# AI-Application-and-Integration-Lab/RDPN6D

Measured on AMD Instinct MI355X. Metric: RGB-D crops/sec (fwd+PnP) at 256x256, higher is better.
Workload: dtype f32

## Files before the change

include/rdpn6d.h:

```cpp
#ifndef RDPN6D_H
#define RDPN6D_H

#ifdef __cplusplus
extern "C" {
#endif

#define RDPN6D_OK 0
#define RDPN6D_EINVAL -1
#define RDPN6D_EHIP -2
#define RDPN6D_ENOMEM -3

const char* rdpn6d_last_error(void);
int rdpn6d_version(void);
int rdpn6d_device_count(void);

void farthest_point_sampling(float* pts, int* idxs, int pn, int sn);
void farthest_point_sampling_init_center(float* pts, int* idxs, int pn, int sn);
int rdpn6d_fps_host(const float* pts, int* idxs, int pn, int sn, int start);
int rdpn6d_fps_device(const float* d_pts, const int* d_offsets, int nobj, int max_pn, int sn, int start,
                      int* d_idxs, float* d_mindist, void* stream);
long long rdpn6d_fps_workspace_bytes(int nobj);
int rdpn6d_fps_device_ws(const float* d_pts, const int* d_offsets, int nobj, int max_pn, int sn, int start, int* d_idxs,
                         float* d_mindist, void* workspace, long long workspace_bytes, void* stream);

// ... 28 lines not shown

int rdpn6d_conv2d_bf16(const rdpn6d_conv_desc* d, int out_f32, void* stream);
int rdpn6d_conv2d_splitk_bf16(const rdpn6d_conv_desc* d, int out_f32, int ksplit, float* workspace, void* stream);
int rdpn6d_conv2d_bf16_bnstats(const rdpn6d_conv_desc* d, double* stats, int stats_row0, int* stats_rows, void* stream);
int rdpn6d_conv2d_bf16_bnbwd(const rdpn6d_conv_desc* d, const void* bn_x, int bn_cs, int bn_co, const float* mean, const float* invstd,
                             const float* gamma, const float* beta, double* partial, int* rows, void* stream);
int rdpn6d_bn_relu_backward_apply_bf16(const void* x, int xcs, int xco, const void* dy, int dcs, int dco, const float* mean,
                                       const float* invstd, const float* gamma, const float* beta, float* dgamma, float* dbeta, void* dx,
                                       int xgcs, int xgco, long long M, int C, const double* partial, int S, void* stream);
int rdpn6d_conv2d_bf16_bnbwd_y(const rdpn6d_conv_desc* d, const void* bn_x, int bn_cs, int bn_co, const void* bn_y, int y_cs, int y_co,
                               const float* mean, const float* invstd, double* partial, int* rows, void* stream);
int rdpn6d_bn_backward_apply_bf16(const void* x, int xcs, int xco, const void* dy, int dcs, int dco, const void* y, int ycs, int yco,
                                  const float* mean, const float* invstd, const float* gamma, float* dgamma, float* dbeta, void* dx,
                                  int xgcs, int xgco, void* dres, int rcs, int rco, long long M, int C, const double* partial, int S,
                                  void* stream);
void rdpn6d_conv_bf16_force_tile(int bm, int bn);
void rdpn6d_conv_bf16_force_stages(int nst);
int rdpn6d_conv_bf16_tile_for(const rdpn6d_conv_desc* d, int* bm, int* bn);
int rdpn6d_conv_bf16_uses_pingpong(const rdpn6d_conv_desc* d, int out_f32);
int rdpn6d_split_bf16x3(const float* x, long long n, void* planes, long long plane_elems, void* stream);
int rdpn6d_conv_bf16x3_eligible(const rdpn6d_conv_desc* d);
int rdpn6d_conv_bf16x3_kernel_for(const rdpn6d_conv_desc* d);
int rdpn6d_conv2d_bf16x3(const rdpn6d_conv_desc* d, long long x_plane_elems, long long w_plane_elems, void* y_planes,
                         long long y_plane_elems, void* stream);
int rdpn6d_conv2d_bf16x3_ex(const rdpn6d_conv_desc* d, long long x_plane_elems, long long w_plane_elems, void* y_planes,
                            long long y_plane_elems, const void* res_planes, long long res_plane_elems, void* stream);
int rdpn6d_split_h2(const float* x, int src_cs, int src_co, int C, void* dst, long long npix, int* overflow_flag, void* stream);
int rdpn6d_conv_h2_kernel_for(const rdpn6d_conv_desc* d);
int rdpn6d_conv2d_h2(const rdpn6d_conv_desc* d, void* y_h2, const void* res_h2, int* overflow_flag, void* stream);
int rdpn6d_conv2d_h2_cb(const rdpn6d_conv_desc* d, void* y_h2, const void* res_h2, int* overflow_flag, const float* crop_bias,
                        void* stream);
long long rdpn6d_conv_h2_workspace_bytes(const rdpn6d_conv_desc* d);
void rdpn6d_conv_h2_set_clock_probe(unsigned long long* buf);
void rdpn6d_conv_h2_set_wfrag(int mode);
int rdpn6d_conv_h2_colmax_ok(const rdpn6d_conv_desc* d, int rows_per_group);
int rdpn6d_conv2d_h2_colmax(const rdpn6d_conv_desc* d, unsigned long long* keys, int rows_per_group, int* overflow_flag, void* stream);
int rdpn6d_h2_colmax_decode(unsigned long long* keys, int groups, int N, int Npad, void* out_h2, void* stream);
int rdpn6d_conv_h2_wfrag_wanted(const rdpn6d_conv_desc* d);
int rdpn6d_h2_weight_frag(const void* w_h2, int Npad, int ntaps, int cchunks, void* w_frag, void* stream);
int rdpn6d_conv2d_h2_wf(const rdpn6d_conv_desc* d, void* y_h2, const void* res_h2, int* overflow_flag, const void* w_frag, void* stream);
int rdpn6d_conv2d_h2_ws(const rdpn6d_conv_desc* d, void* y_h2, const void* res_h2, int* overflow_flag, const float* crop_bias,
                        void* workspace, long long workspace_bytes, void* stream);
int rdpn6d_conv_h2_fuse1x1_ok(const rdpn6d_conv_desc* d);
int rdpn6d_conv2d_h2_fuse1x1(const rdpn6d_conv_desc* d, const void* res_h2, int* overflow_flag, const float* crop_bias,
                             const void* w1_h2, const float* scale1, const float* bias1, float* out, int out_cs, int n_out,
                             void* stream);
int rdpn6d_upsample_bilinear_h2(const void* x, int B, int H, int W, int C, int factor, void* y, int* overflow_flag, void* stream);
int rdpn6d_upsample_bilinear_h2_ex(const void* x, int B, int H, int W, int C, int factor, void* y, int out_cs, int out_co, int relu,
                                   int* overflow_flag, void* stream);
int rdpn6d_xyz_subsample_h2(const float* x, int B, int xc, int R, int step, void* y, int out_cs, int out_co, int* overflow_flag,
                            void* stream);
int rdpn6d_global_max_concat_h2(void* buf, int B, int HW, int C, int cs, void* stream);
int rdpn6d_global_max_h2(const void* x_h2, int B, int HW, int C, int cs, void* gmax_h2, void* stream);
int rdpn6d_convt3x3s2_const_bias_f32(const float* V, const float* scale, int B, int F, float* out , void* stream);
int rdpn6d_stem_pool_h2(const float* x, int B, int xc, int R, const void* w_h2, const float* scale, const float* shift, void* y,
                        int* overflow_flag, void* stream);
int rdpn6d_stem_pool_h2_ex(const float* x, int B, int xc, int R, const void* w_h2, const float* scale, const float* shift, void* y,
                           int out_fmt, int* overflow_flag, void* stream);
int rdpn6d_stem_pack_h2(const float* w_oihw, void* w_h2, float* inv_scale, void* stream);
void rdpn6d_conv_bf16_force_chunk(int row_bytes);
int rdpn6d_stem_conv7x7_bf16(const float* x, int B, int xc, int R, const float* w, const float* scale,
                             const float* shift, void* y, void* stream);
int rdpn6d_maxpool3x3s2_bf16(const void* x, int B, int H, int W, int C, void* y, void* stream);
int rdpn6d_upsample_bilinear_bf16(const void* x, int B, int H, int W, int C, int factor, void* y, void* stream);
int rdpn6d_xyz_subsample_bf16(const float* x, int B, int xc, int R, int step, void* y, int out_cs, int out_co,
                              void* stream);
// ... 281 lines not shown
```

rdpn6d_amd/_lib.py:

```python
import ctypes
import os

HERE = os.path.dirname(os.path.abspath(__file__))
LIB_PATH = os.environ.get("RDPN6D_LIB") or os.path.join(HERE, "librdpn6d_hip.so")

_ll = ctypes.c_longlong
c_float_p = ctypes.c_void_p
c_int_p = ctypes.c_void_p
_vp, _i, _f, _u = ctypes.c_void_p, ctypes.c_int, ctypes.c_float, ctypes.c_uint


class ConvDesc(ctypes.Structure):

    _fields_ = [
        ("x", _vp), ("w", _vp), ("scale", _vp), ("shift", _vp), ("res", _vp), ("y", _vp),
        ("B", _i), ("H", _i), ("W", _i), ("Cin", _i), ("in_cs", _i), ("in_co", _i), ("Ho", _i), ("Wo", _i),
        ("stride", _i), ("ntaps", _i), ("dy", _i * 9), ("dx", _i * 9), ("N", _i), ("Npad", _i), ("OH", _i), ("OW", _i),
        ("osy", _i), ("osx", _i), ("ooy", _i), ("oox", _i), ("out_cs", _i), ("out_co", _i), ("res_cs", _i),
        ("res_co", _i), ("act", _i), ("slope", _f),
    ]


SIGNATURES = {
    "rdpn6d_last_error": (ctypes.c_char_p, []),
# ... 103 lines not shown
    "rdpn6d_bn_train_stats_bf16": (_i, [_vp, _ll, _i, _i, _i, _f, _f, _vp, _vp, _vp, _vp, _vp, _vp]),
    "rdpn6d_bn_apply_bf16": (_i, [_vp, _i, _i, _vp, _vp, _vp, _vp, _vp, _i, _i, _vp, _i, _i, _ll, _i, _i, _vp]),
    "rdpn6d_bn_backward_bf16": (_i, [_vp, _i, _i, _vp, _i, _i, _vp, _i, _i, _vp, _vp, _vp, _vp, _vp, _vp, _i, _i, _vp, _i, _i,
                                     _ll, _i, _i, _vp, _vp]),
    "rdpn6d_bn_relu_backward_bf16": (_i, [_vp, _i, _i, _vp, _i, _i, _vp, _vp, _vp, _vp, _vp, _vp, _vp, _i, _i, _ll, _i, _vp, _vp]),
    "rdpn6d_channel_sum_bf16": (_i, [_vp, _ll, _i, _i, _i, _vp, _i, _vp, _vp]),
    "rdpn6d_maxpool3x3s2_backward_bf16": (_i, [_vp, _vp, _i, _i, _i, _i, _vp, _vp]),
    "rdpn6d_upsample_bilinear_backward_bf16": (_i, [_vp, _i, _i, _i, _i, _i, _vp, _vp]),
    "rdpn6d_global_max_concat_backward_bf16": (_i, [_vp, _vp, _i, _i, _i, _i, _vp, _vp]),
    "rdpn6d_stem_im2col_bf16": (_i, [_vp, _i, _i, _i, _vp, _vp]),
    "rdpn6d_stem_rowpatch_bf16": (_i, [_vp, _i, _i, _i, _vp, _vp]),
    "rdpn6d_repack_f32": (_i, [_vp, _vp, _vp, _i, _vp]),
    "rdpn6d_split_h2": (_i, [_vp, _i, _i, _i, _vp, _ll, _vp, _vp]),
    "rdpn6d_conv_h2_kernel_for": (_i, [_vp]),
    "rdpn6d_conv2d_h2": (_i, [_vp, _vp, _vp, _vp, _vp]),
    "rdpn6d_upsample_bilinear_h2": (_i, [_vp, _i, _i, _i, _i, _i, _vp, _vp, _vp]),
    "rdpn6d_xyz_subsample_h2": (_i, [_vp, _i, _i, _i, _i, _vp, _i, _i, _vp, _vp]),
    "rdpn6d_stem_pool_h2": (_i, [_vp, _i, _i, _i, _vp, _vp, _vp, _vp, _vp, _vp]),
    "rdpn6d_stem_pool_h2_ex": (_i, [_vp, _i, _i, _i, _vp, _vp, _vp, _vp, _i, _vp, _vp]),
    "rdpn6d_stem_pack_h2": (_i, [_vp, _vp, _vp, _vp]),
    "rdpn6d_global_max_concat_h2": (_i, [_vp, _i, _i, _i, _i, _vp]),
    "rdpn6d_upsample_bilinear_h2_ex": (_i, [_vp, _i, _i, _i, _i, _i, _vp, _i, _i, _i, _vp, _vp]),
    "rdpn6d_global_max_h2": (_i, [_vp, _i, _i, _i, _i, _vp, _vp]),
    "rdpn6d_convt3x3s2_const_bias_f32": (_i, [_vp, _vp, _i, _i, _vp, _vp]),
    "rdpn6d_conv2d_h2_cb": (_i, [_vp, _vp, _vp, _vp, _vp, _vp]),
    "rdpn6d_conv2d_h2_ws": (_i, [_vp, _vp, _vp, _vp, _vp, _vp, ctypes.c_longlong, _vp]),
    "rdpn6d_conv_h2_fuse1x1_ok": (_i, [ctypes.POINTER(ConvDesc)]),
    "rdpn6d_conv2d_h2_fuse1x1": (_i, [ctypes.POINTER(ConvDesc), _vp, _vp, _vp, _vp, _vp, _vp, _vp, _i, _i, _vp]),
    "rdpn6d_conv_h2_workspace_bytes": (ctypes.c_longlong, [_vp]),
    "rdpn6d_conv_h2_colmax_ok": (_i, [ctypes.POINTER(ConvDesc), _i]),
    "rdpn6d_conv2d_h2_colmax": (_i, [ctypes.POINTER(ConvDesc), _vp, _i, _vp, _vp]),
    "rdpn6d_h2_colmax_decode": (_i, [_vp, _i, _i, _i, _vp, _vp]),
    "rdpn6d_conv_h2_set_wfrag": (None, [_i]),
    "rdpn6d_conv_h2_set_clock_probe": (None, [_vp]),
    "rdpn6d_conv_h2_wfrag_wanted": (_i, [ctypes.POINTER(ConvDesc)]),
    "rdpn6d_h2_weight_frag": (_i, [_vp, _i, _i, _i, _vp, _vp]),
    "rdpn6d_conv2d_h2_wf": (_i, [ctypes.POINTER(ConvDesc), _vp, _vp, _vp, _vp, _vp]),
    "rdpn6d_ransac_pnp_f32": (_i, [_vp, _vp, _vp, _vp, _vp, _i, _i, _f, _i, _f, ctypes.c_uint, _i, _f, _vp, _vp, _vp, _vp, _vp]),
    "rdpn6d_ransac_pnp_ex": (_i, [_vp, _vp, _vp, _vp, _vp, _i, _i, _f, _i, _f, ctypes.c_uint, _i, _f, _i, _vp, _vp, _vp, _vp, _vp]),
    "rdpn6d_ransac_pnp_workspace_bytes": (_ll, [_i]),
    "rdpn6d_ransac_pnp_ws": (_i, [_vp, _vp, _vp, _vp, _vp, _i, _i, _f, _i, _f, ctypes.c_uint, _i, _f, _i, _vp, _vp, _vp, _vp, _vp, _ll, _vp]),
    "rdpn6d_select_correspondences_f32": (_i, [_vp, _i, _vp, _i, _i, _i, _vp, _vp, _i, _i, _i, _i, _f, _vp, _vp, _vp, _vp, _vp, _vp]),
    "rdpn6d_select_correspondences_mt_f32": (_i, [_vp, _i, _vp, _i, _i, _i, _vp, _vp, _i, _i, _i, _i, _f, _i, _vp, _vp, _vp, _vp, _vp, _vp]),
}

for _k in [k for k in list(SIGNATURES) if "_bf16" in k and "bf16x3" not in k]:
    SIGNATURES[_k.replace("_bf16", "_fp16")] = SIGNATURES[_k]
SIGNATURES["rdpn6d_repack_fp16"] = SIGNATURES["rdpn6d_repack_f32"]

_lib = None


def load():
    global _lib
    if _lib is None:
        if not os.path.exists(LIB_PATH):
            raise RuntimeError(
                f"{LIB_PATH} is missing: build the HIP extension first (python -m rdpn6d_amd.build). "
                "rdpn6d_amd has no CPU fallback."
            )
        import torch

        if torch.cuda.device_count() > 0:
            torch.cuda.init()
        lib = ctypes.CDLL(LIB_PATH)
        for name, (res, args) in SIGNATURES.items():
# ... 12 lines not shown
```

rdpn6d_amd/csrc/conv_igemm_h2.hip:

```cpp
#include "conv_h2_common.h"

#include <cstdio>
#include <cstdlib>

#ifdef RDPN6D_PROBE
__device__ unsigned long long* g_h2_probe = nullptr;
extern "C" int rdpn6d_debug_h2_probe(void* buf)
{
    RD_CHECK_HIP(hipMemcpyToSymbol(HIP_SYMBOL(g_h2_probe), &buf, sizeof(buf)));
    return RDPN6D_OK;
}
#endif

namespace {

constexpr int HT_BYTES = 16384;
constexpr int LDS_8PH = 2 * 4 * HT_BYTES;
constexpr int LDS_8PH_FUSED = 8 * (32 * 72 * 4 + 32 * 272);
static_assert(LDS_8PH_FUSED >= LDS_8PH && LDS_8PH_FUSED <= 160 * 1024, "LDS");

template <bool FUSE, bool CMAX>
__device__ __forceinline__ void conv_h2_8ph_body(const ConvH2Args& ax)
{
    extern __shared__ __attribute__((aligned(1024))) unsigned char smem[];
// ... 412 lines not shown
        const unsigned long long t_issued = __builtin_readcyclecounter();
        asm volatile("s_waitcnt vmcnt(0)" ::: "memory");
        const unsigned long long t_done = __builtin_readcyclecounter();
        if (g_h2_probe && lane == 0) {
            unsigned long long* o = g_h2_probe + ((size_t)blockIdx.x * 8 + wave) * 8;
            o[0] = pq_loop0 - pq_start;
            o[1] = pq_loop1 - pq_loop0;
            o[2] = t_issued - pq_loop1;
            o[3] = t_done - t_issued;
            o[4] = pq_rt0;
            o[5] = __builtin_amdgcn_s_memrealtime();
            o[6] = (unsigned long long)nk;
        }
    }
#endif
}

template <bool FUSE>
__global__ __launch_bounds__(512) void conv_h2_8ph_kernel_t(const ConvH2Args ax)
{
    const bool probe = ax.clk_probe != nullptr && blockIdx.x == 0 && blockIdx.y == 0;
    unsigned long long t0 = 0, r0 = 0;
    if (probe) { t0 = __builtin_readcyclecounter(); r0 = __builtin_amdgcn_s_memrealtime(); }
    conv_h2_8ph_body<FUSE, false>(ax);
    if (probe && threadIdx.x == 0) {
        ax.clk_probe[0] = t0; ax.clk_probe[1] = r0;
        ax.clk_probe[2] = __builtin_readcyclecounter(); ax.clk_probe[3] = __builtin_amdgcn_s_memrealtime();
    }
}
__global__ __launch_bounds__(512) void conv_h2_8ph_colmax_kernel(const ConvH2Args ax) { conv_h2_8ph_body<false, true>(ax); }

constexpr auto conv_h2_8ph_kernel = conv_h2_8ph_kernel_t<false>;

template <int BM, int BN, int NST, int SCHED = 0>
__global__ __launch_bounds__(256, 2) void conv_h2_tile_kernel(const ConvH2Args ax)
{
    constexpr int NW = 4, RB = 128;
    constexpr int RPP = 1024 / RB;
    constexpr int WGN = 2, WTM = BM / 2, WTN = BN / 2;
    constexpr int TM = WTM / 32, TN = WTN / 32;
    constexpr int AG = BM / RPP / NW, BG = BN / RPP / NW;
    constexpr int NDMA = AG + BG;
    static_assert(TM >= 1 && TN >= 1 && AG >= 1 && BG >= 1, "tile / wave layout");
    extern __shared__ __attribute__((aligned(1024))) unsigned char smem[];
    unsigned char* As = smem;
    unsigned char* Bs = smem + NST * BM * RB;

    const ConvBArgs& a = ax.b;
    const rdpn6d_conv_desc& d = a.d;
    const int nblk = a.mtiles * a.ntiles;
    const int bid = blockIdx.x;
    const int q8 = nblk >> 3, r8 = nblk & 7, xcd = bid & 7, kk = bid >> 3;
    const int logical = (xcd < r8 ? xcd * (q8 + 1) : r8 * (q8 + 1) + (xcd - r8) * q8) + kk;
    const int nt = logical % a.ntiles;
    const int mt = logical / a.ntiles;
    const long long m0 = (long long)mt * BM;
    const int n0 = nt * BN;

    const int tid = threadIdx.x;
    const int lane = tid & 63;
    const int wave = __builtin_amdgcn_readfirstlane(tid >> 6);

    const int prow = lane >> 3, pslot = lane & 7;
    const unsigned px_bytes = (unsigned)d.in_cs * 4u;
    unsigned a_base[AG], a_mask[AG];
#pragma unroll
    for (int i = 0; i < AG; ++i) {
        const int row = (wave + NW * i) * RPP + prow;
        const long long m = m0 + row;
        const bool ok = m < a.M;
        const int mm = ok ? (int)m : 0;
        const int b = mm / a.HoWo;
        const int rem = mm - b * a.HoWo;
        const int oy = rem / d.Wo;
        const int ox = rem - oy * d.Wo;
        const int iy = oy * d.stride, ix = ox * d.stride;
        const int lslot = pslot ^ ((row >> 1) & 7);
        a_base[i] = (unsigned)((b * d.H + iy) * d.W + ix) * px_bytes + (unsigned)d.in_co * 4u + (unsigned)lslot * 16u;
        unsigned mask = 0;
        for (int t = 0; t < d.ntaps; ++t) {
            const int dy = (int)((a.dy_pack >> (4 * t)) & 15ull) - 8, dx = (int)((a.dx_pack >> (4 * t)) & 15ull) - 8;
            mask |= (ok && (unsigned)(iy + dy) < (unsigned)d.H && (unsigned)(ix + dx) < (unsigned)d.W) ? (1u << t) : 0u;
        }
        a_mask[i] = mask;
    }
    unsigned w_off[BG];
#pragma unroll
    for (int i = 0; i < BG; ++i) {
        const int row = (wave + NW * i) * RPP + prow;
        const int lslot = pslot ^ ((row >> 1) & 7);
        w_off[i] = (unsigned)(n0 + row) * (unsigned)a.Ktot * 4u + (unsigned)lslot * 16u;
    }
    const __amdgpu_buffer_rsrc_t xsrc = __builtin_amdgcn_make_buffer_rsrc(const_cast<float*>(d.x), 0, a.x_bytes, 0x00020000);
    const __amdgpu_buffer_rsrc_t wsrc = __builtin_amdgcn_make_buffer_rsrc(const_cast<float*>(d.w), 0, a.w_bytes, 0x00020000);

    auto stage_chunk = [&](const int tap, const int cc, const int st) {
        const int dy = (int)((a.dy_pack >> (4 * tap)) & 15ull) - 8, dx = (int)((a.dx_pack >> (4 * tap)) & 15ull) - 8;
        const unsigned toff = (unsigned)((dy * d.W + dx) * (int)px_bytes + cc * RB);
#pragma unroll
        for (int i = 0; i < AG; ++i) {
// ... 66 lines not shown
                rl[i][rr] = f16x8{};
            }
        }
    float scj[TN], shj[TN];
#pragma unroll
    for (int j = 0; j < TN; ++j) {
        const int n = nb + j * 32 + frow;
        scj[j] = (d.scale && !ax.partial) ? d.scale[n] : 1.f;
        shj[j] = (d.shift && !ax.partial) ? d.shift[n] : 0.f;
    }

    f32x16 acc[TM][TN];
#pragma unroll
    for (int i = 0; i < TM; ++i)
#pragma unroll
        for (int j = 0; j < TN; ++j)
#pragma unroll
            for (int e = 0; e < 16; ++e) acc[i][j][e] = 0.f;

    auto mma = [&](const u32x4 (&fa)[TM][4], const u32x4 (&fb)[TN][4]) {
        H2_PAIRS;
#pragma unroll
        for (int pr = 0; pr < 6; ++pr)
#pragma unroll
            for (int i = 0; i < TM; ++i)
#pragma unroll
                for (int jn = 0; jn < TN; ++jn) acc[i][jn] = h2_mfma(fa[i][H2_PA[pr]], fb[jn][H2_PB[pr]], acc[i][jn]);
    };

    u32x4 fa0[TM][4], fb0[TN][4], fa1[TM][4], fb1[TN][4];
    [[maybe_unused]] unsigned long long pr_sum[5] = {0, 0, 0, 0, 0};
    [[maybe_unused]] const unsigned long long pr_start = SCHED == 9 ? __builtin_readcyclecounter() : 0ull;
    [[maybe_unused]] const unsigned long long pr_rt0 = SCHED == 9 ? (__builtin_amdgcn_s_memrealtime() & 0xffffffffull) : 0ull;
    if constexpr (NST == 2) {
        stage_chunk(ld_tap, ld_cc, 0);
        next_chunk(ld_tap, ld_cc, ld_left, d.ntaps);
        stage_chunk(ld_tap, ld_cc, 1);
        next_chunk(ld_tap, ld_cc, ld_left, d.ntaps);
        __syncthreads();
        read_frags(0, fa0, fb0);
        __syncthreads();
        const int npairs = nk >> 1;
        for (int pr = 0; pr < npairs; ++pr) {
            stage_chunk(ld_tap, ld_cc, 0);
            next_chunk(ld_tap, ld_cc, ld_left, d.ntaps);
            read_frags(1, fa1, fb1);
            mma(fa0, fb0);
            __syncthreads();

            stage_chunk(ld_tap, ld_cc, 1);
            next_chunk(ld_tap, ld_cc, ld_left, d.ntaps);
            read_frags(0, fa0, fb0);
            mma(fa1, fb1);
            __syncthreads();
        }
        if (nk & 1) mma(fa0, fb0);
    } else {
        auto publish = [&]() {
            asm volatile("s_waitcnt vmcnt(%0) lgkmcnt(0)" ::"n"(NDMA) : "memory");
            __builtin_amdgcn_s_barrier();
            asm volatile("" ::: "memory");
        };
        stage_chunk(ld_tap, ld_cc, 0);
        next_chunk(ld_tap, ld_cc, ld_left, d.ntaps);
        stage_chunk(ld_tap, ld_cc, 1);
        next_chunk(ld_tap, ld_cc, ld_left, d.ntaps);
        stage_chunk(ld_tap, ld_cc, 2);
// ... 62 lines not shown
        const int hi = lane >> 5;
        asm volatile("s_waitcnt vmcnt(0) lgkmcnt(0)" ::: "memory");
        __builtin_amdgcn_s_barrier();
        asm volatile("" ::: "memory");
        float* cst = reinterpret_cast<float*>(smem) + wave * (32 * CS);
        if (ax.partial) {
            float* part = ax.partial + ((size_t)blockIdx.y * ax.mpad + (size_t)m0 + wm * WTM) * d.Npad + nb + c8;
#pragma unroll
            for (int i = 0; i < TM; ++i) {
#pragma unroll
                for (int j = 0; j < TN; ++j)
#pragma unroll
                    for (int e = 0; e < 16; ++e) cst[((e & 3) + 8 * (e >> 2) + 4 * hi) * CS + j * 32 + frow] = acc[i][j][e];
#pragma unroll
                for (int rr = 0; rr < 32 / RPI; ++rr) {
                    const int row = rr * RPI + rrow;
                    float* pp = part + (size_t)(i * 32 + row) * d.Npad;
                    *reinterpret_cast<f32x4*>(pp) = *reinterpret_cast<const f32x4*>(cst + row * CS + c8);
                    *reinterpret_cast<f32x4*>(pp + 4) = *reinterpret_cast<const f32x4*>(cst + row * CS + c8 + 4);
                }
            }
            return;
        }
#pragma unroll
        for (int i = 0; i < TM; ++i) {
#pragma unroll
            for (int j = 0; j < TN; ++j)
#pragma unroll
                for (int e = 0; e < 16; ++e)
                    cst[((e & 3) + 8 * (e >> 2) + 4 * hi) * CS + j * 32 + frow] = acc[i][j][e] * scj[j] + shj[j];
#pragma unroll
            for (int rr = 0; rr < NRR; ++rr) {
                const int row = rr * RPI + rrow;
                if (pixs[i][rr] >= 0) {
                    const f32x4 lo = *reinterpret_cast<const f32x4*>(cst + row * CS + c8);
                    const f32x4 hi4 = *reinterpret_cast<const f32x4*>(cst + row * CS + c8 + 4);
                    float v[8] = {lo[0], lo[1], lo[2], lo[3], hi4[0], hi4[1], hi4[2], hi4[3]};
                    if (res_pre) h2_finish_row8_t<true>(ax, v, pixs[i][rr], nb + c8, rh[i][rr], rl[i][rr]);
                    else h2_finish_row8_t<false>(ax, v, pixs[i][rr], nb + c8, rh[i][rr], rl[i][rr]);
                }
            }
        }
    }
#ifdef RDPN6D_PROBE
    if constexpr (SCHED == 9) {
        if (g_h2_probe && lane == 0) {
            const unsigned long long t_end = __builtin_readcyclecounter();
            unsigned long long* o = g_h2_probe + ((size_t)blockIdx.x * 4 + wave) * 8;
            for (int i = 0; i < 5; ++i) o[i] = pr_sum[i];
            o[5] = pr_loop_end - pr_start;
            o[6] = t_end - pr_loop_end;
            o[7] = pr_rt0 | (__builtin_amdgcn_s_memrealtime() << 32);
        }
    }
#endif
}

__global__ __launch_bounds__(256) void h2_splitk_reduce_kernel(const ConvH2Args ax)
{
    const ConvBArgs& a = ax.b;
    const rdpn6d_conv_desc& d = a.d;
    const int n8 = d.Npad >> 3;
    const long long total = a.M * n8;
    const size_t sstride = (size_t)ax.mpad * d.Npad;
    for (long long i = (long long)blockIdx.x * 256 + threadIdx.x; i < total; i += (long long)gridDim.x * 256) {
        const long long m = i / n8;
        const int ch = (int)(i - m * n8) * 8;
        if (ch >= d.N) continue;
        const float* pp = ax.partial + (size_t)m * d.Npad + ch;
        f32x4 s0 = *reinterpret_cast<const f32x4*>(pp), s1 = *reinterpret_cast<const f32x4*>(pp + 4);
        int sl = 1;
        for (; sl + 3 <= ax.nsplit; sl += 3) {
// ... 15 lines not shown
            v[q] = s0[q] * (d.scale ? d.scale[ch + q] : 1.f) + (d.shift ? d.shift[ch + q] : 0.f);
            v[4 + q] = s1[q] * (d.scale ? d.scale[ch + 4 + q] : 1.f) + (d.shift ? d.shift[ch + 4 + q] : 0.f);
        }
        h2_finish_row8(ax, v, h2_pixel_of(a, m), ch);
    }
}

template <int BM, int BN, int NST, int SCHED = 0>
int launch_h2_tile_s(const ConvH2Args& ax, hipStream_t s);
template <int BM, int BN, int NST>
int launch_h2_tile(const ConvH2Args& ax, hipStream_t s)
{
#ifdef RDPN6D_PROBE
    static const int sched = getenv("RDPN6D_H2_SCHED") ? atoi(getenv("RDPN6D_H2_SCHED")) : 0;
    if (sched == 9) return launch_h2_tile_s<BM, BN, NST, 9>(ax, s);
#endif
    return launch_h2_tile_s<BM, BN, NST, 0>(ax, s);
}
template <int BM, int BN, int NST, int SCHED>
int launch_h2_tile_s(const ConvH2Args& ax, hipStream_t s)
{
    constexpr int lds_stage = NST * (BM + BN) * 128;
    constexpr int lds_epi = 4 * 32 * (BN / 2 + 8) * 4;
    constexpr int lds = lds_stage > lds_epi ? lds_stage : lds_epi;
    static_assert(lds <= 80 * 1024 || (BM == 128 && BN == 128 && NST == 3), "two workgroups per CU (128x128 with three stages: one)");
    auto kern = conv_h2_tile_kernel<BM, BN, NST, SCHED>;
    if (lds > 64 * 1024) {
        RD_LDS_OPT_IN(kern, lds);
    }
    hipLaunchKernelGGL(kern, dim3((unsigned)(ax.b.mtiles * ax.b.ntiles), (unsigned)ax.nsplit), dim3(256), lds, s, ax);
    return RDPN6D_OK;
}

__global__ void split_h2_kernel(const float* __restrict__ x, int src_cs, int src_co, int C, _Float16* __restrict__ dst, long long npix,
                                int* __restrict__ overflow_flag)
{
    const int c8n = C >> 3;
    const long long total = npix * c8n;
    bool over = false;
    for (long long i = (long long)blockIdx.x * blockDim.x + threadIdx.x; i < total; i += (long long)gridDim.x * blockDim.x) {
        const long long p = i / c8n;
        const int c = (int)(i - p * c8n) * 8;
        const float* sp = x + p * src_cs + src_co + c;
        const f32x4 v0 = *reinterpret_cast<const f32x4*>(sp), v1 = *reinterpret_cast<const f32x4*>(sp + 4);
        const float v[8] = {v0[0], v0[1], v0[2], v0[3], v1[0], v1[1], v1[2], v1[3]};
        f16x8 hi, lo;
        float sv[8];
#pragma unroll
        for (int q = 0; q < 8; ++q) sv[q] = v[q] * H2_SCALE;
        over |= h2_split8(sv, hi, lo);
        _Float16* pp = dst + p * (2 * (long long)C) + (c >> 5) * 64 + (c & 31);
        *reinterpret_cast<f16x8*>(pp) = hi;
        *reinterpret_cast<f16x8*>(pp + 32) = lo;
    }
    if (over && overflow_flag) *overflow_flag = 1;
}

bool h2_common_ok(const rdpn6d_conv_desc* d)
{
    return d->Cin % 32 == 0 && d->in_cs % 32 == 0 && d->in_co % 32 == 0 && d->out_cs % 8 == 0 && d->out_co % 8 == 0 && d->N % 8 == 0 &&
           d->Npad % 64 == 0 && (!d->res || (d->res_cs % 4 == 0 && d->res_co % 4 == 0));
}
bool h2_big_ok(const rdpn6d_conv_desc* d)
{
    const int nk = d->ntaps * (d->Cin / 32);
    return h2_common_ok(d) && d->Npad % 256 == 0 && d->N == d->Npad && nk >= 2 && (nk & 1) == 0;
// ... 37 lines not shown

static int h2_pp_plan(const rdpn6d_conv_desc* d, long long M, int* pbm, int* pbn)
{
    static const int on = getenv("RDPN6D_H2_PP") ? atoi(getenv("RDPN6D_H2_PP")) : 1;
    static const int force = getenv("RDPN6D_H2_PP_SHAPE") ? atoi(getenv("RDPN6D_H2_PP_SHAPE")) : -1;
    if (!on || d->Npad % 128 != 0 || d->ntaps * (d->Cin / 32) < 8) return -1;
    int shape = 0;
    if ((long long)rd_cdiv(M, 256) * (d->Npad / 128) >= 224 && (long long)rd_cdiv(M, 128) * (d->Npad / 128) > 288) shape = 2;
    if (force == 0 || force == 2) shape = force;
    const int bm = shape == 0 ? 128 : 256;
    if ((long long)rd_cdiv(M, bm) * (d->Npad / 128) < 224) return -1;
    *pbm = bm;
    *pbn = 128;
    return shape;
}

static int h2_tile_ksplit(const rdpn6d_conv_desc* d, long long M, int bm, int bn)
{
    static const int off = getenv("RDPN6D_H2_NO_SPLITK") ? 1 : 0;
    const long long tiles = (long long)rd_cdiv(M, bm) * (d->Npad / bn);
    static const int tmax = getenv("RDPN6D_H2_SPLIT_TILES") ? atoi(getenv("RDPN6D_H2_SPLIT_TILES")) : 128;
    if (off || tiles >= tmax) return 0;
    const int nk = d->ntaps * (d->Cin / 32);
    int best = 0;
    for (int sl = 2; sl <= 32; sl *= 2)
        if (tiles * sl <= 512 && nk % sl == 0 && nk / sl >= 4) best = sl;
    return best;
}

static int g_h2_wfrag_mode = getenv("RDPN6D_H2_BFG") ? atoi(getenv("RDPN6D_H2_BFG")) : 0;
extern "C" void rdpn6d_conv_h2_set_wfrag(int mode) { g_h2_wfrag_mode = mode; }
static unsigned long long* g_h2_clk_probe = nullptr;
extern "C" void rdpn6d_conv_h2_set_clock_probe(unsigned long long* buf) { g_h2_clk_probe = buf; }
static bool h2_wfrag_shape_ok(int shape)
{
    const int mode = g_h2_wfrag_mode;
    return mode >= 1 && (shape == 0 || (mode >= 2 && shape == 2));
}

extern "C" int rdpn6d_conv_h2_kernel_for(const rdpn6d_conv_desc* d)
{
    if (!d || !h2_common_ok(d)) return 0;
    const long long M = (long long)d->B * d->Ho * d->Wo;
    return (h2_big_ok(d) && h2_big_pays(d, M)) ? 2 : 1;
}

extern "C" int rdpn6d_conv2d_h2_cb(const rdpn6d_conv_desc* d, void* y_h2, const void* res_h2, int* overflow_flag, const float* crop_bias,
                                   void* stream);
extern "C" int rdpn6d_conv2d_h2(const rdpn6d_conv_desc* d, void* y_h2, const void* res_h2, int* overflow_flag, void* stream)
{
    return rdpn6d_conv2d_h2_cb(d, y_h2, res_h2, overflow_flag, nullptr, stream);
}

extern "C" long long rdpn6d_conv_h2_workspace_bytes(const rdpn6d_conv_desc* d)
{
    if (!d || rdpn6d_conv_h2_kernel_for(d) != 1) return 0;
    const long long M = (long long)d->B * d->Ho * d->Wo;
    int bm, bn;
    if (h2_pp_plan(d, M, &bm, &bn) >= 0) return 0;
    h2_pick_tile(d, M, &bm, &bn);
    return (long long)h2_tile_ksplit(d, M, bm, bn) * rd_cdiv(M, bm) * bm * d->Npad * 4;
}

extern "C" int rdpn6d_conv2d_h2_ws(const rdpn6d_conv_desc* d, void* y_h2, const void* res_h2, int* overflow_flag, const float* crop_bias,
                                   void* workspace, long long workspace_bytes, void* stream);
extern "C" int rdpn6d_conv2d_h2_cb(const rdpn6d_conv_desc* d, void* y_h2, const void* res_h2, int* overflow_flag, const float* crop_bias,
                                   void* stream)
{
    return rdpn6d_conv2d_h2_ws(d, y_h2, res_h2, overflow_flag, crop_bias, nullptr, 0, stream);
}

struct H2Fuse {
    const void* w;
    const float *scale, *bias;
    float* out;
    int cs, n;
};
// ... 146 lines not shown
    for (int t = 0; t < d->ntaps; ++t) {
        RD_REQUIRE(d->dy[t] >= -8 && d->dy[t] <= 7 && d->dx[t] >= -8 && d->dx[t] <= 7, "tap offsets must be in -8..7");
        a.dy_pack |= (unsigned long long)(d->dy[t] + 8) << (4 * t);
        a.dx_pack |= (unsigned long long)(d->dx[t] + 8) << (4 * t);
    }
    a.kper = a.nk;
    a.partial = nullptr;
    hipStream_t s = (hipStream_t)stream;
    if (which == 1) {
        int bm, bn;
        const int shape = h2_pp_plan(d, a.M, &bm, &bn);
        if (shape >= 0) {
            a.mtiles = rd_cdiv(a.M, bm);
            a.ntiles = d->Npad / bn;
            ax.w_frag = h2_wfrag_shape_ok(shape) ? w_frag : nullptr;
            const int rc = conv_h2_launch_pp(ax, shape, s);
            if (rc != RDPN6D_OK) return rc;
            RD_LAUNCH_CHECK();
            return RDPN6D_OK;
        }
        h2_pick_tile(d, a.M, &bm, &bn);
        a.mtiles = rd_cdiv(a.M, bm);
        a.ntiles = d->Npad / bn;
        const int ks = h2_tile_ksplit(d, a.M, bm, bn);
        if (ks && workspace && workspace_bytes >= (long long)ks * a.mtiles * bm * d->Npad * 4) {
            ax.nsplit = ks;
            ax.mpad = a.mtiles * bm;
            ax.partial = reinterpret_cast<float*>(workspace);
            a.kper = a.nk / ks;
        }
        int rc;
        static const int nst_env = getenv("RDPN6D_H2_NST") ? atoi(getenv("RDPN6D_H2_NST")) : 0;
        const bool three = nst_env ? nst_env == 3 : a.kper >= 32;
        if (bm == 128 && bn == 128) rc = (nst_env == 3) ? launch_h2_tile<128, 128, 3>(ax, s) : launch_h2_tile<128, 128, 2>(ax, s);
        else if (bm == 128) rc = three ? launch_h2_tile<128, 64, 3>(ax, s) : launch_h2_tile<128, 64, 2>(ax, s);
        else if (bn == 128) rc = three ? launch_h2_tile<64, 128, 3>(ax, s) : launch_h2_tile<64, 128, 2>(ax, s);
        else rc = three ? launch_h2_tile<64, 64, 3>(ax, s) : launch_h2_tile<64, 64, 2>(ax, s);
        if (rc != RDPN6D_OK) return rc;
        RD_LAUNCH_CHECK();
        if (ax.partial) {
            const long long items = a.M * (d->Npad / 8);
            hipLaunchKernelGGL(h2_splitk_reduce_kernel, dim3((unsigned)((items + 255) / 256 < 4096 ? (items + 255) / 256 : 4096)), dim3(256), 0, s, ax);
            RD_LAUNCH_CHECK();
        }
        return RDPN6D_OK;
    }
    a.mtiles = rd_cdiv(a.M, 256);
    a.ntiles = d->Npad / 256;
    if (fuse && !fuse->w) {
        RD_LDS_OPT_IN(conv_h2_8ph_colmax_kernel, LDS_8PH);
        hipLaunchKernelGGL(conv_h2_8ph_colmax_kernel, dim3((unsigned)(a.mtiles * a.ntiles)), dim3(512), LDS_8PH, s, ax);
        RD_LAUNCH_CHECK();
        return RDPN6D_OK;
    }
    if (fuse) {
        RD_LDS_OPT_IN(conv_h2_8ph_kernel_t<true>, LDS_8PH_FUSED);
        hipLaunchKernelGGL(conv_h2_8ph_kernel_t<true>, dim3((unsigned)(a.mtiles * a.ntiles)), dim3(512), LDS_8PH_FUSED, s, ax);
        RD_LAUNCH_CHECK();
        return RDPN6D_OK;
    }
    RD_LDS_OPT_IN(conv_h2_8ph_kernel, LDS_8PH);
#ifdef RDPN6D_PROBE
    if (const char* e = getenv("RDPN6D_H2_ABL_A")) ax.nsplit = 100 + atoi(e);
#endif
    hipLaunchKernelGGL(conv_h2_8ph_kernel, dim3((unsigned)(a.mtiles * a.ntiles)), dim3(512), LDS_8PH, s, ax);
    RD_LAUNCH_CHECK();
// ... 3 lines not shown
```

Baseline: 9186.

## Add halo-patch staging path for 3x3 stride-1 fp16 conv tiles

Adds a patch-based variant of the tiled implicit-GEMM conv kernel for 3x3 stride-1 convs on narrow feature maps (W of 8 or 16, 64x64 tiles). For each channel chunk it loads one halo patch of input rows into double-buffered LDS, and all nine taps read shifted fragments from it, with x-boundary masking applied in registers. This replaces re-staging the A operand once per tap, cutting global loads. The cost is a more complex pipeline, per-tap masking work, and recomputing pixel indices in the epilogue.

```diff
diff --git a/include/rdpn6d.h b/include/rdpn6d.h
--- a/include/rdpn6d.h
+++ b/include/rdpn6d.h
@@ -84,6 +84,8 @@
                         void* stream);
 long long rdpn6d_conv_h2_workspace_bytes(const rdpn6d_conv_desc* d);
 void rdpn6d_conv_h2_set_clock_probe(unsigned long long* buf);
+void rdpn6d_conv_h2_set_patch(int on);
+int rdpn6d_conv_h2_patch_for(const rdpn6d_conv_desc* d);
 void rdpn6d_conv_h2_set_wfrag(int mode);
 int rdpn6d_conv_h2_colmax_ok(const rdpn6d_conv_desc* d, int rows_per_group);
 int rdpn6d_conv2d_h2_colmax(const rdpn6d_conv_desc* d, unsigned long long* keys, int rows_per_group, int* overflow_flag, void* stream);
diff --git a/rdpn6d_amd/_lib.py b/rdpn6d_amd/_lib.py
--- a/rdpn6d_amd/_lib.py
+++ b/rdpn6d_amd/_lib.py
@@ -159,6 +159,8 @@
     "rdpn6d_conv2d_h2_colmax": (_i, [ctypes.POINTER(ConvDesc), _vp, _i, _vp, _vp]),
     "rdpn6d_h2_colmax_decode": (_i, [_vp, _i, _i, _i, _vp, _vp]),
     "rdpn6d_conv_h2_set_wfrag": (None, [_i]),
+    "rdpn6d_conv_h2_set_patch": (None, [_i]),
+    "rdpn6d_conv_h2_patch_for": (_i, [ctypes.POINTER(ConvDesc)]),
     "rdpn6d_conv_h2_set_clock_probe": (None, [_vp]),
     "rdpn6d_conv_h2_wfrag_wanted": (_i, [ctypes.POINTER(ConvDesc)]),
     "rdpn6d_h2_weight_frag": (_i, [_vp, _i, _i, _i, _vp, _vp]),
diff --git a/rdpn6d_amd/csrc/conv_igemm_h2.hip b/rdpn6d_amd/csrc/conv_igemm_h2.hip
--- a/rdpn6d_amd/csrc/conv_igemm_h2.hip
+++ b/rdpn6d_amd/csrc/conv_igemm_h2.hip
@@ -468,7 +468,7 @@
 
 constexpr auto conv_h2_8ph_kernel = conv_h2_8ph_kernel_t<false>;
 
-template <int BM, int BN, int NST, int SCHED = 0>
+template <int BM, int BN, int NST, int SCHED = 0, int PW = 0>
 __global__ __launch_bounds__(256, 2) void conv_h2_tile_kernel(const ConvH2Args ax)
 {
     constexpr int NW = 4, RB = 128;
@@ -479,8 +479,9 @@
     constexpr int NDMA = AG + BG;
     static_assert(TM >= 1 && TN >= 1 && AG >= 1 && BG >= 1, "tile / wave layout");
     extern __shared__ __attribute__((aligned(1024))) unsigned char smem[];
+    constexpr int PB = PW * NW * 1024;
     unsigned char* As = smem;
-    unsigned char* Bs = smem + NST * BM * RB;
+    unsigned char* Bs = smem + (PW > 0 ? 2 * PB : NST * BM * RB);
 
     const ConvBArgs& a = ax.b;
     const rdpn6d_conv_desc& d = a.d;
@@ -499,9 +500,9 @@
 
     const int prow = lane >> 3, pslot = lane & 7;
     const unsigned px_bytes = (unsigned)d.in_cs * 4u;
-    unsigned a_base[AG], a_mask[AG];
-#pragma unroll
-    for (int i = 0; i < AG; ++i) {
+    unsigned a_base[AG] = {}, a_mask[AG] = {};
+#pragma unroll
+    for (int i = 0; i < (PW > 0 ? 0 : AG); ++i) {
         const int row = (wave + NW * i) * RPP + prow;
         const long long m = m0 + row;
         const bool ok = m < a.M;
@@ -634,7 +635,153 @@
     [[maybe_unused]] unsigned long long pr_sum[5] = {0, 0, 0, 0, 0};
     [[maybe_unused]] const unsigned long long pr_start = SCHED == 9 ? __builtin_readcyclecounter() : 0ull;
     [[maybe_unused]] const unsigned long long pr_rt0 = SCHED == 9 ? (__builtin_amdgcn_s_memrealtime() & 0xffffffffull) : 0ull;
-    if constexpr (NST == 2) {
+    if constexpr (PW > 0) {
+        constexpr int PN = PW > 0 ? PW : 1;
+        const int W = d.W;
+        const int y0 = (int)(m0 % a.HoWo) / W;
+        const bool top = y0 > 0, bot = y0 + BM / W < d.H;
+        unsigned p_off[PN];
+#pragma unroll
+        for (int i = 0; i < PN; ++i) {
+            const int p = (wave + NW * i) * RPP + prow;
+            const bool ok = p < BM + 2 * W && (p >= W || top) && (p < BM + W || bot);
+            const int lslot = pslot ^ ((p >> 1) & 7);
+            p_off[i] = ok ? (unsigned)(int)(m0 - W + p) * px_bytes + (unsigned)d.in_co * 4u + (unsigned)lslot * 16u : 0xFFFFFFFFu;
+        }
+        const int cc_last = a.cchunks - 1;
+        auto stage_patch = [&](auto ic_, const int cc, const int par) {
+            constexpr int i = decltype(ic_)::value;
+            const int cs = __builtin_amdgcn_readfirstlane((cc < cc_last ? cc : cc_last) * RB);
+            unsigned char* dst = As + par * PB + (wave + NW * i) * 1024;
+            __builtin_amdgcn_raw_ptr_buffer_load_lds(xsrc, (lds_ptr_t)dst, 16, (int)p_off[i], cs, 0, 0);
+        };
+        auto stage_patch_step = [&](auto tc, const int cc, const int par) {
+            constexpr int t = decltype(tc)::value;
+            if constexpr (t < 7) {
+                if constexpr (t < PW) stage_patch(ic<t>{}, cc, par);
+                if constexpr (t + 7 < PW) stage_patch(ic<t + 7>{}, cc, par);
+            }
+            static_assert(PW <= 14, "patch pieces per wave");
+        };
+        const int cin4 = d.Cin * 4;
+        auto stage_w = [&](const int tap, const int cc, const int st) {
+            const bool past = cc > cc_last;
+            const int wk = __builtin_amdgcn_readfirstlane((past ? 8 : tap) * cin4 + (past ? cc_last : cc) * RB);
+#pragma unroll
+            for (int i = 0; i < BG; ++i) {
+                unsigned char* dst = Bs + ((st * BN) + (wave + NW * i) * RPP) * RB;
+                __builtin_amdgcn_raw_ptr_buffer_load_lds(wsrc, (lds_ptr_t)dst, 16, (int)w_off[i], wk, 0, 0);
+            }
+        };
+        unsigned fa_p[9][TM], m_neg[TM], m_pos[TM];
+#pragma unroll
+        for (int i = 0; i < TM; ++i) {
+            const int R = wm * WTM + i * 32 + frow;
+            const int x = R % W;
+            m_neg[i] = x > 0 ? 0xFFFFFFFFu : 0u;
+            m_pos[i] = x < W - 1 ? 0xFFFFFFFFu : 0u;
+#pragma unroll
+            for (int t = 0; t < 9; ++t) {
+                const int dy = t / 3 - 1, dx = t % 3 - 1;
+                const bool in = dx < 0 ? x > 0 : (dx > 0 ? x < W - 1 : true);
+                const int p = R + W + (in ? dy * W + dx : 0);
+                fa_p[t][i] = ((unsigned)p << 7) | ((unsigned)(((p >> 1) & 7) ^ half) << 4);
+            }
+        }
+        auto read_frags_p = [&](auto tc, auto parc, const int st, u32x4 (&fa)[TM][4], u32x4 (&fb)[TN][4]) {
+            constexpr int t = decltype(tc)::value, par = decltype(parc)::value;
+            const unsigned char* pa = As + par * PB;
+#pragma unroll
+            for (int i = 0; i < TM; ++i) {
+                unsigned base = fa_p[t][i];
+                asm volatile("" : "+v"(base));
+#pragma unroll
+                for (int j = 0; j < 4; ++j) fa[i][j] = *reinterpret_cast<const u32x4*>(pa + (base ^ (unsigned)(j << 5)));
+            }
+#pragma unroll
+            for (int jn = 0; jn < TN; ++jn) {
+                const int R = wn * WTN + jn * 32 + frow;
+                const int sw = (R >> 1) & 7;
+                const unsigned char* q = Bs + ((st * BN) + R) * RB;
+#pragma unroll
+                for (int j = 0; j < 4; ++j) fb[jn][j] = *reinterpret_cast<const u32x4*>(q + (((2 * j + half) ^ sw) << 4));
+            }
+        };
+        auto mask_frags = [&](auto tc, u32x4 (&fa)[TM][4]) {
+            constexpr int dx = decltype(tc)::value % 3 - 1;
+            if constexpr (dx != 0) {
+#pragma unroll
+                for (int i = 0; i < TM; ++i) {
+                    const unsigned m = dx < 0 ? m_neg[i] : m_pos[i];
+#pragma unroll
+                    for (int j = 0; j < 4; ++j) fa[i][j] &= u32x4{m, m, m, m};
+                }
+            }
+        };
+        stage_patch_step(ic<0>{}, 0, 0);
+        stage_patch_step(ic<1>{}, 0, 0);
+        stage_patch_step(ic<2>{}, 0, 0);
+        stage_patch_step(ic<3>{}, 0, 0);
+        stage_patch_step(ic<4>{}, 0, 0);
+        stage_patch_step(ic<5>{}, 0, 0);
+        stage_patch_step(ic<6>{}, 0, 0);
+#pragma unroll
+        for (int st = 0; st < NST; ++st) stage_w(st, 0, st);
+        asm volatile("s_waitcnt vmcnt(%0)" ::"n"((NST - 1) * BG) : "memory");
+        __builtin_amdgcn_s_barrier();
+        asm volatile("" ::: "memory");
+        read_frags_p(ic<0>{}, ic<0>{}, 0, fa0, fb0);
+        asm volatile("s_waitcnt vmcnt(%0) lgkmcnt(0)" ::"n"((NST - 2) * BG) : "memory");
+        __builtin_amdgcn_s_barrier();
+        asm volatile("" ::: "memory");
+        int st_free = 0, st_next = 1;
+        auto pstep = [&](auto tc, auto parc, const int cc, u32x4 (&fcur_a)[TM][4], u32x4 (&fcur_b)[TN][4], u32x4 (&fnxt_a)[TM][4], u32x4 (&fnxt_b)[TN][4]) {
+            constexpr int t = decltype(tc)::value, par = decltype(parc)::value;
+            constexpr int ppt = t < 7 ? ((t < PW ? 1 : 0) + (t + 7 < PW ? 1 : 0)) : 0;
+            stage_w((t + NST) % 9, cc + (t + NST) / 9, st_free);
+            stage_patch_step(tc, cc + 1, par ^ 1);
+            read_frags_p(ic<(t == 8 ? 0 : t + 1)>{}, ic<(t == 8 ? par ^ 1 : par)>{}, st_next, fnxt_a, fnxt_b);
+            __builtin_amdgcn_sched_barrier(0);
+            mask_frags(tc, fcur_a);
+            mma(fcur_a, fcur_b);
+            asm volatile("s_waitcnt vmcnt(%0) lgkmcnt(0)" ::"n"((NST == 2 ? 0 : BG) + ppt) : "memory");
+            __builtin_amdgcn_s_barrier();
+            asm volatile("" ::: "memory");
+            st_free = st_next;
+            st_next = st_next == NST - 1 ? 0 : st_next + 1;
+        };
+        auto pgroup = [&](auto parc, const int cc) {
+            constexpr int par = decltype(parc)::value;
+            if constexpr (par == 0) {
+                pstep(ic<0>{}, parc, cc, fa0, fb0, fa1, fb1);
+                pstep(ic<1>{}, parc, cc, fa1, fb1, fa0, fb0);
+                pstep(ic<2>{}, parc, cc, fa0, fb0, fa1, fb1);
+                pstep(ic<3>{}, parc, cc, fa1, fb1, fa0, fb0);
+                pstep(ic<4>{}, parc, cc, fa0, fb0, fa1, fb1);
+                pstep(ic<5>{}, parc, cc, fa1, fb1, fa0, fb0);
+                pstep(ic<6>{}, parc, cc, fa0, fb0, fa1, fb1);
+                pstep(ic<7>{}, parc, cc, fa1, fb1, fa0, fb0);
+                pstep(ic<8>{}, parc, cc, fa0, fb0, fa1, fb1);
+            } else {
+                pstep(ic<0>{}, parc, cc, fa1, fb1, fa0, fb0);
+                pstep(ic<1>{}, parc, cc, fa0, fb0, fa1, fb1);
+                pstep(ic<2>{}, parc, cc, fa1, fb1, fa0, fb0);
+                pstep(ic<3>{}, parc, cc, fa0, fb0, fa1, fb1);
+                pstep(ic<4>{}, parc, cc, fa1, fb1, fa0, fb0);
+                pstep(ic<5>{}, parc, cc, fa0, fb0, fa1, fb1);
+                pstep(ic<6>{}, parc, cc, fa1, fb1, fa0, fb0);
+                pstep(ic<7>{}, parc, cc, fa0, fb0, fa1, fb1);
+                pstep(ic<8>{}, parc, cc, fa1, fb1, fa0, fb0);
+            }
+        };
+        int cc = 0;
+        for (; cc + 2 <= a.cchunks; cc += 2) {
+            pgroup(ic<0>{}, cc);
+            pgroup(ic<1>{}, cc + 1);
+        }
+        if (cc < a.cchunks) pgroup(ic<0>{}, cc);
+        asm volatile("s_waitcnt vmcnt(0)" ::: "memory");
+    } else if constexpr (NST == 2) {
         stage_chunk(ld_tap, ld_cc, 0);
         next_chunk(ld_tap, ld_cc, ld_left, d.ntaps);
         stage_chunk(ld_tap, ld_cc, 1);
@@ -763,12 +910,17 @@
 #pragma unroll
             for (int rr = 0; rr < NRR; ++rr) {
                 const int row = rr * RPI + rrow;
-                if (pixs[i][rr] >= 0) {
+                long long pix = pixs[i][rr];
+                if constexpr (PW > 0) {
+                    const long long mrow = m0 + wm * WTM + i * 32 + row;
+                    pix = (mrow < a.M && nb + c8 < d.N) ? h2_pixel_of(a, mrow) : -1;
+                }
+                if (pix >= 0) {
                     const f32x4 lo = *reinterpret_cast<const f32x4*>(cst + row * CS + c8);
                     const f32x4 hi4 = *reinterpret_cast<const f32x4*>(cst + row * CS + c8 + 4);
                     float v[8] = {lo[0], lo[1], lo[2], lo[3], hi4[0], hi4[1], hi4[2], hi4[3]};
-                    if (res_pre) h2_finish_row8_t<true>(ax, v, pixs[i][rr], nb + c8, rh[i][rr], rl[i][rr]);
-                    else h2_finish_row8_t<false>(ax, v, pixs[i][rr], nb + c8, rh[i][rr], rl[i][rr]);
+                    if (res_pre) h2_finish_row8_t<true>(ax, v, pix, nb + c8, rh[i][rr], rl[i][rr]);
+                    else h2_finish_row8_t<false>(ax, v, pix, nb + c8, rh[i][rr], rl[i][rr]);
                 }
             }
         }
@@ -850,6 +1002,21 @@
     return RDPN6D_OK;
 }
 
+template <int BM, int BN, int NST, int PW>
+int launch_h2_tile_patch(const ConvH2Args& ax, hipStream_t s)
+{
+    constexpr int lds_stage = 2 * PW * 4096 + NST * BN * 128;
+    constexpr int lds_epi = 4 * 32 * (BN / 2 + 8) * 4;
+    constexpr int lds = lds_stage > lds_epi ? lds_stage : lds_epi;
+    static_assert(lds <= 80 * 1024, "two workgroups per CU");
+    auto kern = conv_h2_tile_kernel<BM, BN, NST, 0, PW>;
+    if (lds > 64 * 1024) {
+        RD_LDS_OPT_IN(kern, lds);
+    }
+    hipLaunchKernelGGL(kern, dim3((unsigned)(ax.b.mtiles * ax.b.ntiles), 1u), dim3(256), lds, s, ax);
+    return RDPN6D_OK;
+}
+
 __global__ void split_h2_kernel(const float* __restrict__ x, int src_cs, int src_co, int C, _Float16* __restrict__ dst, long long npix,
                                 int* __restrict__ overflow_flag)
 {
@@ -953,6 +1120,16 @@
 extern "C" void rdpn6d_conv_h2_set_wfrag(int mode) { g_h2_wfrag_mode = mode; }
 static unsigned long long* g_h2_clk_probe = nullptr;
 extern "C" void rdpn6d_conv_h2_set_clock_probe(unsigned long long* buf) { g_h2_clk_probe = buf; }
+static int g_h2_patch = getenv("RDPN6D_H2_PATCH") ? atoi(getenv("RDPN6D_H2_PATCH")) : 1;
+extern "C" void rdpn6d_conv_h2_set_patch(int on) { g_h2_patch = on; }
+static bool h2_patch_ok(const rdpn6d_conv_desc* d, int bm, int bn, bool split_or_bias)
+{
+    if (!g_h2_patch || split_or_bias || d->ntaps != 9 || d->stride != 1 || d->H != d->Ho || d->W != d->Wo) return false;
+    for (int t = 0; t < 9; ++t)
+        if (d->dy[t] != t / 3 - 1 || d->dx[t] != t % 3 - 1) return false;
+    if (bn != 64 || bm % d->W != 0 || (d->H * d->W) % bm != 0) return false;
+    return bm == 64 && (d->W == 8 || d->W == 16);
+}
 static bool h2_wfrag_shape_ok(int shape)
 {
     const int mode = g_h2_wfrag_mode;
@@ -964,6 +1141,16 @@
     if (!d || !h2_common_ok(d)) return 0;
     const long long M = (long long)d->B * d->Ho * d->Wo;
     return (h2_big_ok(d) && h2_big_pays(d, M)) ? 2 : 1;
+}
+
+extern "C" int rdpn6d_conv_h2_patch_for(const rdpn6d_conv_desc* d)
+{
+    if (!d || rdpn6d_conv_h2_kernel_for(d) != 1) return 0;
+    const long long M = (long long)d->B * d->Ho * d->Wo;
+    int bm, bn;
+    if (h2_pp_plan(d, M, &bm, &bn) >= 0) return 0;
+    h2_pick_tile(d, M, &bm, &bn);
+    return h2_patch_ok(d, bm, bn, false) ? 1 : 0;
 }
 
 extern "C" int rdpn6d_conv2d_h2_cb(const rdpn6d_conv_desc* d, void* y_h2, const void* res_h2, int* overflow_flag, const float* crop_bias,
@@ -1176,6 +1363,9 @@
         int rc;
         static const int nst_env = getenv("RDPN6D_H2_NST") ? atoi(getenv("RDPN6D_H2_NST")) : 0;
         const bool three = nst_env ? nst_env == 3 : a.kper >= 32;
+        if (h2_patch_ok(d, bm, bn, ax.partial || ax.crop_bias)) {
+            rc = three ? launch_h2_tile_patch<64, 64, 3, 3>(ax, s) : launch_h2_tile_patch<64, 64, 2, 3>(ax, s);
+        } else
         if (bm == 128 && bn == 128) rc = (nst_env == 3) ? launch_h2_tile<128, 128, 3>(ax, s) : launch_h2_tile<128, 128, 2>(ax, s);
         else if (bm == 128) rc = three ? launch_h2_tile<128, 64, 3>(ax, s) : launch_h2_tile<128, 64, 2>(ax, s);
         else if (bn == 128) rc = three ? launch_h2_tile<64, 128, 3>(ax, s) : launch_h2_tile<64, 128, 2>(ax, s);
```

Result: no change. 9254, median of 6 (+0.7%).
